# kvas7andy/unreal

Measured on NVIDIA B200. Metric: maze env-steps/s incl. pixel-change+returns, higher is better.
Workload: dtype f32

## Files before the change

include/unreal_b200.h:

```cpp
#ifndef UNREAL_B200_H_
#define UNREAL_B200_H_

#include <stdint.h>

#ifdef __cplusplus
extern "C" {
#endif

#define UNREAL_OK 0
#define UNREAL_EINVAL (-1)
#define UNREAL_ECUDA (-2)
#define UNREAL_ESTATE (-3)
#define UNREAL_ENOMEM (-4)

#define UNREAL_F32 0
#define UNREAL_U8 1
#define UNREAL_BF16 2

#define UNREAL_MAZE_GRID 7
#define UNREAL_FRAME_HW 84
#define UNREAL_PC_CELLS 20
#define UNREAL_MT_WORDS 624

const char* unreal_last_error(void);
int unreal_abi_version(void);
int unreal_device_info(int* sm_count, int* cc_major, int* cc_minor);
int unreal_set_tunable(const char* name, int value);
int unreal_get_tunable(const char* name, int* value);

int unreal_maze_set_map(const char* map49_host);
int unreal_maze_get_layout(int* start_x, int* start_y, int* goal_x, int* goal_y, uint8_t* walls49_host);

int unreal_maze_reset(int32_t* pos , int32_t* last_action , float* last_reward ,
                      const uint8_t* mask , int n, void* stream);

int unreal_maze_step(int32_t* pos, const int32_t* action , const uint8_t* active,
                     float* reward , uint8_t* terminal , int32_t* last_action,
                     float* last_reward, void* obs, int obs_dtype, float* pc, uint64_t* frame_rec,
                     int n, int auto_reset, void* stream);

int unreal_maze_window(int32_t* pos, const int32_t* action, float* reward, uint8_t* terminal, int32_t* last_action,
                       float* last_reward, void* obs, int obs_dtype, float* pc, uint64_t* frame_rec, int n, int t,
                       int auto_reset, void* stream);

int unreal_maze_render(const int32_t* pos, void* obs, int obs_dtype, int m, void* stream);

int unreal_maze_pixel_change(const int32_t* pos0, const int32_t* pos1, float* pc, int m, void* stream);
int unreal_maze_pc_targets(const int32_t* pos0, const int32_t* pos1, const int32_t* len, const float* boot, float gamma_pc,
                           float* tgt, int t, int n, void* stream);

int unreal_pixel_change(const void* cur, const void* prev, int dtype, float* pc, int m, int h, int w,
                        int c, void* stream);
int unreal_selfcheck_arith(unsigned long long* mismatches, void* stream);
int unreal_subsample(const float* a, float* out, int m, int h, int w, int width, void* stream);
int unreal_pixel_change_stream(const void* frames, int dtype, float* pc, int s, int l, int h, int w,
                               int c, void* stream);

int unreal_nstep_returns(const float* r, const float* v, const uint8_t* term, const float* boot,
                         float gamma, float* out_R, float* out_adv, int t, int n, void* stream);
int unreal_sequence_returns(const float* r, const int32_t* len, const float* boot, float gamma,
                            float* out_R , int n, int l, void* stream);

int unreal_pc_targets(const float* pc, const uint8_t* term, const int32_t* len, const float* boot,
                      float gamma_pc, float* tgt, int t, int n, void* stream);

int unreal_mt_seed(uint32_t* mt, int32_t* mt_pos, const uint32_t* seeds , int n, void* stream);
int unreal_choose_action(uint32_t* mt, int32_t* mt_pos, const float* pi, const uint8_t* active,
                         int32_t* action, int n, int a, void* stream);
int unreal_mt_randint(uint32_t* mt, int32_t* mt_pos, uint32_t high, int32_t* out, int n, int k, void* stream);

typedef struct unreal_replay unreal_replay_t;
int unreal_replay_create(unreal_replay_t** out, int n_envs, int history_size);
int unreal_replay_destroy(unreal_replay_t* r);
int unreal_replay_reset(unreal_replay_t* r, void* stream);
int unreal_replay_add(unreal_replay_t* r, const uint64_t* frame_rec , void* stream);
int unreal_replay_state(unreal_replay_t* r, uint8_t* full, int32_t* count, int64_t* top,
                        int32_t* n_pos, int32_t* n_neg, void* stream);
int unreal_replay_copy(unreal_replay_t* r, int direction, uint64_t* rec, int64_t* top, int32_t* count,
                       int32_t* n_pos, int32_t* n_neg, void* stream);
int unreal_replay_sample_sequence(unreal_replay_t* r, uint32_t* mt, int32_t* mt_pos, int seq_len,
                                  int32_t* start, int32_t* len, uint64_t* rec, void* stream);
int unreal_replay_sample_rp(unreal_replay_t* r, uint32_t* mt, int32_t* mt_pos, int32_t* start,
                            uint64_t* rec, void* stream);
int unreal_frame_unpack(const uint64_t* rec, int m, int32_t* pos0, int32_t* pos1, int32_t* action,
                        float* reward, uint8_t* terminal, int32_t* last_action, float* last_reward,
                        uint8_t* valid, void* stream);

int unreal_frame_pack(const int32_t* action, const float* reward, const uint8_t* terminal,
                      const int32_t* last_action , const float* last_reward ,
                      const uint8_t* active , uint64_t* rec, int n, void* stream);
int unreal_replay_add_slots(unreal_replay_t* r, const uint64_t* frame_rec, int32_t* slot, void* stream);
int unreal_ring_store(void* payload, const void* src, const int32_t* slot, int n_envs, int history_size,
                      long long item_bytes, void* stream);
int unreal_rows_select(void* out, const void* src, const int64_t* idx, const uint8_t* mask, int n, long long item_bytes,
                       void* stream);
int unreal_replay_gather(unreal_replay_t* r, const void* payload, long long item_bytes, const int32_t* start,
                         const int32_t* len , int seq_len, int time_major, void* out, void* stream);

int unreal_rollout_lar(const int32_t* last_action, const float* last_reward, const float* objective, int n, int a, int g,
                       float* lar, void* stream);
int unreal_rollout_post(const float* reward, const uint8_t* terminal, const uint64_t* frame_rec, int n, uint8_t* active,
                        uint8_t* ended, uint64_t* last_rec, float* episode_reward, float* lstm_c, float* lstm_h,
                        double* stats, void* stream);

int unreal_grad_sumsq(const float* grad, int64_t p, double* sumsq, void* stream);
int unreal_rmsprop_update(float* var, float* rms, float* mom, const float* grad, int64_t p,
                          const double* sumsq, float grad_scale, float lr, float decay, float momentum,
                          float eps, float clip_norm, float* grad_norm, void* stream);
int unreal_rmsprop_update_dlr(float* var, float* rms, float* mom, const float* grad, int64_t p,
                              const double* sumsq, float grad_scale, const float* lr_dev, float decay, float momentum,
                              float eps, float clip_norm, float* grad_norm, void* stream);

#define UNREAL_GEMM_OUT_F32 0
#define UNREAL_GEMM_OUT_BF16 1
int unreal_gemm_bf16(const void* a, int64_t lda, int a_mn_major, const void* b, int64_t ldb, int b_mn_major,
                     void* c, int64_t ldc, int c_dtype, const float* bias, const float* add, int relu,
                     int accumulate, int split_k, int m, int n, int k, void* stream);

int unreal_im2col(const void* in, int in_dtype, void* out_bf16, int s, int h, int w, int c, int kh, int kw,
                  int stride, void* stream);
int unreal_col2im(const void* cols, int cols_dtype, void* out, int out_dtype, const float* bias, int relu, int s,
                  int h, int w, int c, int kh, int kw, int stride, void* stream);
int unreal_lstm_cell_fwd(float* gates, const float* c_prev, float* c_out, float* h_out, void* h16_out, int n,
                         void* stream);
int unreal_lstm_cell_fwd_ld(float* gates, const float* c_prev, float* c_out, float* h_out, void* h16_out, int h16_ld,
                            int n, void* stream);
// ... 82 lines not shown
```

unreal_b200/_lib.py:

```python
import ctypes
import os
from ctypes import POINTER, c_char_p, c_double, c_float, c_int, c_int32, c_int64, c_uint8, c_uint32, c_void_p

import torch

HERE = os.path.dirname(os.path.abspath(__file__))
LIB_PATH = os.path.join(HERE, "libunreal_b200.so")

OK = 0
F32 = 0
U8 = 1


class UnrealError(RuntimeError):
  pass


if not os.path.exists(LIB_PATH):
  raise ImportError(
      "%s is missing: build it with `python -m unreal_b200.build` (nvcc, sm_100a). "
      "unreal_b200 has no CPU fallback." % LIB_PATH)

lib = ctypes.CDLL(LIB_PATH)

P = c_void_p

SIGNATURES = {
    "unreal_last_error": (c_char_p, []),
    "unreal_abi_version": (c_int, []),
    "unreal_device_info": (c_int, [POINTER(c_int), POINTER(c_int), POINTER(c_int)]),
    "unreal_set_tunable": (c_int, [c_char_p, c_int]),
    "unreal_get_tunable": (c_int, [c_char_p, POINTER(c_int)]),
    "unreal_maze_set_map": (c_int, [c_char_p]),
    "unreal_maze_get_layout": (c_int, [POINTER(c_int)] * 4 + [POINTER(c_uint8)]),
    "unreal_maze_reset": (c_int, [P, P, P, P, c_int, P]),
    "unreal_maze_step": (c_int, [P, P, P, P, P, P, P, P, c_int, P, P, c_int, c_int, P]),
    "unreal_maze_window": (c_int, [P, P, P, P, P, P, P, c_int, P, P, c_int, c_int, c_int, P]),
    "unreal_maze_render": (c_int, [P, P, c_int, c_int, P]),
    "unreal_maze_pixel_change": (c_int, [P, P, P, c_int, P]),
    "unreal_maze_pc_targets": (c_int, [P, P, P, P, c_float, P, c_int, c_int, P]),
    "unreal_pixel_change": (c_int, [P, P, c_int, P, c_int, c_int, c_int, c_int, P]),
    "unreal_pixel_change_stream": (c_int, [P, c_int, P, c_int, c_int, c_int, c_int, c_int, P]),
    "unreal_selfcheck_arith": (c_int, [P, P]),
    "unreal_subsample": (c_int, [P, P, c_int, c_int, c_int, c_int, P]),
    "unreal_nstep_returns": (c_int, [P, P, P, P, c_float, P, P, c_int, c_int, P]),
    "unreal_sequence_returns": (c_int, [P, P, P, c_float, P, c_int, c_int, P]),
    "unreal_pc_targets": (c_int, [P, P, P, P, c_float, P, c_int, c_int, P]),
    "unreal_mt_seed": (c_int, [P, P, P, c_int, P]),
    "unreal_choose_action": (c_int, [P, P, P, P, P, c_int, c_int, P]),
    "unreal_mt_randint": (c_int, [P, P, c_uint32, P, c_int, c_int, P]),
    "unreal_replay_create": (c_int, [POINTER(c_void_p), c_int, c_int]),
    "unreal_replay_destroy": (c_int, [c_void_p]),
    "unreal_replay_reset": (c_int, [c_void_p, P]),
    "unreal_replay_add": (c_int, [c_void_p, P, P]),
    "unreal_replay_state": (c_int, [c_void_p, P, P, P, P, P, P]),
    "unreal_replay_copy": (c_int, [c_void_p, c_int, P, P, P, P, P, P]),
    "unreal_replay_sample_sequence": (c_int, [c_void_p, P, P, c_int, P, P, P, P]),
    "unreal_replay_sample_rp": (c_int, [c_void_p, P, P, P, P, P]),
    "unreal_frame_unpack": (c_int, [P, c_int, P, P, P, P, P, P, P, P, P]),
    "unreal_frame_pack": (c_int, [P, P, P, P, P, P, P, c_int, P]),
    "unreal_replay_add_slots": (c_int, [c_void_p, P, P, P]),
    "unreal_ring_store": (c_int, [P, P, P, c_int, c_int, c_int64, P]),
    "unreal_rows_select": (c_int, [P, P, P, P, c_int, c_int64, P]),
    "unreal_replay_gather": (c_int, [c_void_p, P, c_int64, P, P, c_int, c_int, P, P]),
    "unreal_rollout_lar": (c_int, [P, P, P, c_int, c_int, c_int, P, P]),
    "unreal_rollout_post": (c_int, [P, P, P, c_int, P, P, P, P, P, P, P, P]),
    "unreal_grad_sumsq": (c_int, [P, c_int64, P, P]),
    "unreal_rmsprop_update": (c_int, [P, P, P, P, c_int64, P, c_float, c_float, c_float, c_float, c_float,
                                      c_float, P, P]),
    "unreal_rmsprop_update_dlr": (c_int, [P, P, P, P, c_int64, P, c_float, P, c_float, c_float, c_float,
                                          c_float, P, P]),
    "unreal_gemm_bf16": (c_int, [P, c_int64, c_int, P, c_int64, c_int, P, c_int64, c_int, P, P, c_int, c_int, c_int,
                                 c_int, c_int, c_int, P]),
    "unreal_im2col": (c_int, [P, c_int, P, c_int, c_int, c_int, c_int, c_int, c_int, c_int, P]),
    "unreal_col2im": (c_int, [P, c_int, P, c_int, P, c_int, c_int, c_int, c_int, c_int, c_int, c_int, c_int, P]),
    "unreal_lstm_cell_fwd": (c_int, [P, P, P, P, P, c_int, P]),
    "unreal_lstm_cell_fwd_ld": (c_int, [P, P, P, P, P, c_int, c_int, P]),
    "unreal_lstm_cell_act": (c_int, [P, P, P, P, P, c_int, P]),
    "unreal_lstm_cell_fwd_g16": (c_int, [P, P, P, P, P, c_int, c_int, P]),
    "unreal_lstm_cell_act_g16": (c_int, [P, P, P, P, P, c_int, P]),
    "unreal_lstm_cell_act_heads": (c_int, [P, P, P, P, c_int, P, P, P, P, c_int, P, P, P]),
    "unreal_lstm_cell_bwd_g16": (c_int, [P, P, P, P, P, P, P, c_int, P]),
    "unreal_lstm_step_fwd": (c_int, [P, c_int64, P, P, P, P, P, P, P, c_int, P, P, c_int, c_int, c_int, P]),
    "unreal_lstm_step_bwd": (c_int, [P, P, c_int64, P, P, P, P, P, P, P, c_int, c_int, P]),
    "unreal_lstm_cell_bwd": (c_int, [P, P, P, P, P, P, c_int, P]),
    "unreal_lstm_cell_bwd2": (c_int, [P, P, P, P, P, P, P, c_int, P]),
    "unreal_s2d_frames": (c_int, [P, c_int, P, c_int, P]),
    "unreal_conv_fwd": (c_int, [P, c_int, P, P, P, c_int, P]),
    "unreal_relu_grad": (c_int, [P, c_int, P, P, P, c_int64, c_int, c_int, P]),
    "unreal_conv1_wgrad": (c_int, [P, P, P, c_int, P]),
    "unreal_conv2_wgrad": (c_int, [P, P, P, c_int, P]),
    "unreal_conv2_wgrad_c8": (c_int, [P, P, P, c_int, P]),
    "unreal_conv2_dgrad": (c_int, [P, P, P, c_int, P]),
    "unreal_pc_deconv_fwd": (c_int, [P, P, P, P, c_int, P]),
    "unreal_conv2_dgrad_relu": (c_int, [P, P, P, P, P, c_int, c_int, P]),
    "unreal_conv1_wgrad_p21": (c_int, [P, P, P, c_int, P]),
    "unreal_conv1_fwd_maze": (c_int, [P, P, P, P, c_int, P]),
    "unreal_conv1_wgrad_maze": (c_int, [P, P, P, c_int, P]),
    "unreal_a3c_head_loss": (c_int, [P, P, P, P, P, P, P, P, P, c_int64, c_int, c_float, c_float, P, P, P, P, P, P]),
    "unreal_a3c_head_bwd": (c_int, [P, P, P, P, P, P, c_int64, c_int, P, P, P, P, P, P]),
    "unreal_pc_loss": (c_int, [P, P, P, P, c_int, c_float, c_int64, c_int, P, P, P, P]),
    "unreal_pc_loss_grad16": (c_int, [P, P, P, P, c_int, c_float, c_int64, c_int, P, P, P, P]),
    "unreal_cell_gather": (c_int, [P, P, P, c_int64, c_int64, c_int, P]),
    "unreal_cell_segment_sum": (c_int, [P, c_int, P, P, c_int64, c_int, P]),
    "unreal_pc_deconv_loss": (c_int, [P, P, P, P, P, P, c_int, c_float, c_int, P, P, P, P]),
    "unreal_pc_deconv_loss_c8": (c_int, [P, P, P, P, P, P, c_int, c_float, c_int, P, P, P, P]),
    "unreal_pc_deconv_loss_planes": (c_int, [P, P, P, P, P, P, c_int, c_float, c_int, P, P, P, P]),
    "unreal_pc_planes_conv": (c_int, [P, P, P, P, P, P, c_int, P]),
    "unreal_pc_planes_wgrad": (c_int, [P, P, P, c_int, P]),
    "unreal_pc_deconv_qmax": (c_int, [P, P, P, c_int, c_int, P, P]),
    "unreal_conv2_fwd_linear_scaled": (c_int, [P, P, P, P, c_int, P]),
    "unreal_conv2_fwd_linear_masked": (c_int, [P, c_int, P, P, P, P, P, c_int, P]),
    "unreal_rp_loss": (c_int, [P, P, P, c_int64, P, P, P, P, P, P]),
    "unreal_conv2_fwd_linear": (c_int, [P, P, P, c_int, P]),
}

MISSING = []
for _name, (_res, _args) in SIGNATURES.items():
  try:
    _fn = getattr(lib, _name)
# ... 83 lines not shown
```

unreal_b200/csrc/maze.cu:

```cuda
#include "common.cuh"
#include "maze_core.cuh"

namespace unreal {

__constant__ MazeLayout c_maze;
static MazeLayout h_maze;
static bool h_maze_ready = false;

static const char kReferenceMap[] =
    "--+---G"
    "--+-+++"
    "S-+---+"
    "--+++--"
    "--+-+--"
    "--+----"
    "-----++";

constexpr int kFrameElems = UNREAL_FRAME_HW * UNREAL_FRAME_HW * 3;
constexpr int kRowElems = UNREAL_FRAME_HW * 3;
constexpr int kPcElems = UNREAL_PC_CELLS * UNREAL_PC_CELLS;
constexpr int kThreads = 256;

struct StepArgs {
  int32_t* pos;
// ... 363 lines not shown
  const EnvInfo f = window_logic(a, e, t, lane);
  if (a.pc != nullptr) {
    float* pc = a.pc + b * kPcElems;
#pragma unroll
    for (int q = lane; q < kPcElems / 4; q += 32) write_pc(pc, f, q);
  }
  if (a.obs == nullptr) return;
  constexpr int G = Chunk<T>::kGroupsPerBand;
  constexpr int kChunksPerGroup = 63;
  const ChunkMasks m0 = make_masks<T>(lane);
  const ChunkMasks m1 = make_masks<T>(lane + 32);
  const bool has1 = lane + 32 < kChunksPerGroup;
  uint4* out = reinterpret_cast<uint4*>(reinterpret_cast<T*>(a.obs) + b * kFrameElems) + lane;
#pragma unroll
  for (int cy = 0; cy < UNREAL_MAZE_GRID; ++cy) {
    const uint32_t walls = c_maze.wall_rows[cy];
    const uint4 v0 = band_value(m0, walls, cy == f.ry, f.rx);
    const uint4 v1 = band_value(m1, walls, cy == f.ry, f.rx);
#pragma unroll
    for (int g = 0; g < G; ++g) {
      uint4* p = out + (size_t)(cy * G + g) * kChunksPerGroup;
      __stcs(p, v0);
      if (has1) __stcs(p + 32, v1);
    }
  }
}

template <typename T, int kWarps>
__global__ void __launch_bounds__(kWarps * 32) maze_window_env_kernel(WindowArgs a, int32_t* pos_out, int32_t* la_out,
                                                                      float* lr_out) {
  const int lane = threadIdx.x & 31;
  const int e = blockIdx.x * kWarps + (threadIdx.x >> 5);
  if (e >= a.n) return;
  constexpr int G = Chunk<T>::kGroupsPerBand;
  constexpr int kChunksPerGroup = 63;
  const ChunkMasks m0 = make_masks<T>(lane);
  const ChunkMasks m1 = make_masks<T>(lane + 32);
  const bool has1 = lane + 32 < kChunksPerGroup;
  uint4 w0[UNREAL_MAZE_GRID], w1[UNREAL_MAZE_GRID];
#pragma unroll
  for (int cy = 0; cy < UNREAL_MAZE_GRID; ++cy) {
    w0[cy] = band_value(m0, c_maze.wall_rows[cy], false, 0);
    w1[cy] = band_value(m1, c_maze.wall_rows[cy], false, 0);
  }
  const int mine = (lane < a.t) ? a.action[(size_t)lane * a.n + e] : 0;
  MazeCursor c{a.pos[2 * e], a.pos[2 * e + 1], a.last_action[e], a.last_reward[e]};
  for (int t = 0; t < a.t; ++t) {
    const int act = __shfl_sync(0xffffffffu, mine, t);
    const MazeStep st = maze_step_core(c_maze, c.x, c.y, act);
    const size_t b = (size_t)t * a.n + e;
    if (lane == 0) {
      if (a.rec) a.rec[b] = frame_pack(c.x, c.y, st.x1, st.y1, act, st.reward, st.terminal, c.la, (int)c.lr);
      a.reward[b] = (float)st.reward;
      a.terminal[b] = (uint8_t)st.terminal;
    }
    EnvInfo f;
    f.x0 = c.x; f.y0 = c.y; f.x1 = st.x1; f.y1 = st.y1; f.live = 1;
    cursor_advance(c, st, act, a.auto_reset);
    f.rx = c.x; f.ry = c.y;
    if (a.pc != nullptr) {
      float* pc = a.pc + b * kPcElems;
#pragma unroll
      for (int q = lane; q < kPcElems / 4; q += 32) write_pc(pc, f, q);
    }
    if (a.obs == nullptr) continue;
    uint4* out = reinterpret_cast<uint4*>(reinterpret_cast<T*>(a.obs) + b * kFrameElems) + lane;
    const uint4 ag0 = band_value(m0, 0u, true, f.rx), ag1 = band_value(m1, 0u, true, f.rx);
#pragma unroll
    for (int cy = 0; cy < UNREAL_MAZE_GRID; ++cy) {
      uint4 v0 = w0[cy], v1 = w1[cy];
      if (cy == f.ry) {
        v0.x |= ag0.x; v0.y |= ag0.y; v0.z |= ag0.z; v0.w |= ag0.w;
        v1.x |= ag1.x; v1.y |= ag1.y; v1.z |= ag1.z; v1.w |= ag1.w;
      }
#pragma unroll
      for (int g = 0; g < G; ++g) {
        uint4* p = out + (size_t)(cy * G + g) * kChunksPerGroup;
        __stcs(p, v0);
        if (has1) __stcs(p + 32, v1);
      }
    }
  }
  if (lane == 0) { pos_out[2 * e] = c.x; pos_out[2 * e + 1] = c.y; la_out[e] = c.la; lr_out[e] = c.lr; }
}

template <bool kStep>
__global__ void __launch_bounds__(256) maze_s2d_kernel(StepArgs a) {
  __shared__ EnvInfo s_info;
  const int tid = threadIdx.x;
  const int e = blockIdx.x;
  if (tid == 0) s_info = env_logic<kStep>(a, e);
  __syncthreads();
  const EnvInfo f = s_info;
  if (!f.live) return;
  if (a.pc != nullptr && tid >= 256 - kPcElems / 4) write_pc(a.pc + (size_t)e * kPcElems, f, tid - (256 - kPcElems / 4));
  if (a.obs == nullptr) return;
  uint4* out = reinterpret_cast<uint4*>(a.obs) + (size_t)e * (6 * 441);
  int kind[2];
#pragma unroll
  for (int h = 0; h < 2; ++h) {
    const int pix = tid + h * 256;
    const int Y = pix / 21, X = pix - Y * 21;
    const int cx = X / 3, cy = Y / 3;
    kind[h] = pix < 441 ? (int)((c_maze.wall_rows[cy] >> cx) & 1u) | (((cx == f.rx) && (cy == f.ry)) ? 2 : 0) : -1;
  }
#pragma unroll
  for (int q = 0; q < 6; ++q) {
    const int base = (2 * q) % 3;
    uint32_t wl[4], ag[4];
#pragma unroll
    for (int k = 0; k < 4; ++k) {
      const int c0 = (base + 2 * k) % 3, c1 = (base + 2 * k + 1) % 3;
      wl[k] = (c0 == 0 ? 0x3f80u : 0u) | (c1 == 0 ? 0x3f800000u : 0u);
      ag[k] = (c0 == 1 ? 0x3f80u : 0u) | (c1 == 1 ? 0x3f800000u : 0u);
    }
#pragma unroll
    for (int h = 0; h < 2; ++h) {
      if (kind[h] < 0) continue;
      const uint32_t mw = (kind[h] & 1) ? 0xffffffffu : 0u, ma = (kind[h] & 2) ? 0xffffffffu : 0u;
      __stcs(out + q * 441 + tid + h * 256, make_uint4((wl[0] & mw) | (ag[0] & ma), (wl[1] & mw) | (ag[1] & ma),
                                                       (wl[2] & mw) | (ag[2] & ma), (wl[3] & mw) | (ag[3] & ma)));
    }
  }
}

__global__ void __launch_bounds__(128) maze_pc_pairs_kernel(const int32_t* __restrict__ p0,
                                                            const int32_t* __restrict__ p1, float* pc, int m) {
  int idx = blockIdx.x * blockDim.x + threadIdx.x;
  int e = idx / (kPcElems / 4), q = idx - e * (kPcElems / 4);
  if (e >= m) return;
  EnvInfo f;
  f.x0 = p0[2 * e]; f.y0 = p0[2 * e + 1]; f.x1 = p1[2 * e]; f.y1 = p1[2 * e + 1];
  f.rx = f.ry = 0; f.live = 1;
  write_pc(pc + (size_t)e * kPcElems, f, q);
}

__global__ void __launch_bounds__(128) maze_pc_targets_kernel(const int2* __restrict__ p0, const int2* __restrict__ p1,
                                                              const int32_t* __restrict__ len, const float4* __restrict__ boot,
                                                              float g, float4* __restrict__ tgt, int T, int N) {
  const size_t per_t = (size_t)N * (kPcElems / 4);
  const size_t idx = (size_t)blockIdx.x * 128 + threadIdx.x;
  if (idx >= per_t) return;
  const int n = (int)(idx / (kPcElems / 4)), q = (int)(idx - (size_t)n * (kPcElems / 4));
  const int n_t = len ? max(0, min(len[n], T)) : T;
  const float4 zero = make_float4(0.f, 0.f, 0.f, 0.f);
  float4 R = boot[idx];
  for (int t = T - 1; t >= n_t; --t) __stcs(tgt + (size_t)t * per_t + idx, zero);
#pragma unroll 4
  for (int t = n_t - 1; t >= 0; --t) {
    const int2 a = __ldg(p0 + (size_t)t * N + n), b = __ldg(p1 + (size_t)t * N + n);
    const float4 pc = pc_value4(a.x, a.y, b.x, b.y, q);
    R.x = __fadd_rn(pc.x, __fmul_rn(g, R.x));
    R.y = __fadd_rn(pc.y, __fmul_rn(g, R.y));
    R.z = __fadd_rn(pc.z, __fmul_rn(g, R.z));
    R.w = __fadd_rn(pc.w, __fmul_rn(g, R.w));
    __stcs(tgt + (size_t)t * per_t + idx, R);
  }
}

__global__ void maze_reset_kernel(int32_t* pos, int32_t* last_action, float* last_reward, const uint8_t* mask,
                                  int n) {
  int e = blockIdx.x * blockDim.x + threadIdx.x;
  if (e >= n || (mask != nullptr && mask[e] == 0)) return;
  pos[2 * e] = c_maze.start_x;
  pos[2 * e + 1] = c_maze.start_y;
  if (last_action) last_action[e] = 0;
// ... 140 lines not shown
  if (rc) return rc;
  StepArgs a{pos, action, active, reward, terminal, last_action, last_reward, obs, pc, frame_rec, n, auto_reset};
  return launch_render<true>(a, obs_dtype, as_stream(stream));
}

extern "C" int unreal_maze_render(const int32_t* pos, void* obs, int obs_dtype, int m, void* stream) {
  UNREAL_REQUIRE(pos && obs && m >= 0, "unreal_maze_render: null argument or m < 0");
  UNREAL_REQUIRE(obs_dtype == UNREAL_F32 || obs_dtype == UNREAL_U8 || obs_dtype == UNREAL_BF16,
                 "unreal_maze_render: bad obs_dtype %d", obs_dtype);
  UNREAL_REQUIRE(aligned16(obs), "unreal_maze_render: obs must be 16-byte aligned");
  int rc = ensure_map();
  if (rc) return rc;
  StepArgs a{const_cast<int32_t*>(pos), nullptr, nullptr, nullptr, nullptr, nullptr, nullptr, obs, nullptr, nullptr, m, 0};
  return launch_render<false>(a, obs_dtype, as_stream(stream));
}

extern "C" int unreal_maze_pixel_change(const int32_t* pos0, const int32_t* pos1, float* pc, int m, void* stream) {
  UNREAL_REQUIRE(pos0 && pos1 && pc && m >= 0, "unreal_maze_pixel_change: null argument or m < 0");
  UNREAL_REQUIRE(aligned16(pc), "unreal_maze_pixel_change: pc must be 16-byte aligned");
  if (m == 0) return UNREAL_OK;
  long long threads = (long long)m * (kPcElems / 4);
  maze_pc_pairs_kernel<<<(unsigned)((threads + 127) / 128), 128, 0, as_stream(stream)>>>(pos0, pos1, pc, m);
  UNREAL_LAUNCH_CHECK("maze_pc_pairs_kernel");
  return UNREAL_OK;
}

extern "C" int unreal_maze_pc_targets(const int32_t* pos0, const int32_t* pos1, const int32_t* len, const float* boot,
                                      float gamma_pc, float* tgt, int t, int n, void* stream) {
  UNREAL_REQUIRE(t >= 0 && n >= 0, "unreal_maze_pc_targets: negative size");
  if (t == 0 || n == 0) return UNREAL_OK;
  UNREAL_REQUIRE(pos0 && pos1 && boot && tgt, "unreal_maze_pc_targets: pos0, pos1, boot and tgt must be non-null");
  UNREAL_REQUIRE(aligned16(boot) && aligned16(tgt) && (reinterpret_cast<uintptr_t>(pos0) & 7u) == 0 &&
                 (reinterpret_cast<uintptr_t>(pos1) & 7u) == 0, "unreal_maze_pc_targets: alignment (16 bytes; cells 8)");
  const long long cols = (long long)n * (kPcElems / 4);
  maze_pc_targets_kernel<<<(unsigned)((cols + 127) / 128), 128, 0, as_stream(stream)>>>(
      reinterpret_cast<const int2*>(pos0), reinterpret_cast<const int2*>(pos1), len, reinterpret_cast<const float4*>(boot),
      gamma_pc, reinterpret_cast<float4*>(tgt), t, n);
  UNREAL_LAUNCH_CHECK("maze_pc_targets_kernel");
  return UNREAL_OK;
}

extern "C" int unreal_maze_window(int32_t* pos, const int32_t* action, float* reward, uint8_t* terminal, int32_t* last_action,
                                  float* last_reward, void* obs, int obs_dtype, float* pc, uint64_t* frame_rec, int n, int t,
                                  int auto_reset, void* stream) {
  UNREAL_REQUIRE(n >= 0 && t >= 0, "unreal_maze_window: negative size");
  UNREAL_REQUIRE(t <= 32, "unreal_maze_window: at most 32 steps per window (got %d)", t);
  UNREAL_REQUIRE(pos && action && reward && terminal && last_action && last_reward,
                 "unreal_maze_window: pos/action/reward/terminal/last_action/last_reward must be non-null");
  UNREAL_REQUIRE(obs_dtype == UNREAL_F32 || obs_dtype == UNREAL_U8, "unreal_maze_window: obs_dtype must be f32 or u8");
  UNREAL_REQUIRE(aligned16(obs) && aligned16(pc), "unreal_maze_window: obs and pc must be 16-byte aligned");
  UNREAL_REQUIRE((long long)n * t < 2147483647LL / 4, "unreal_maze_window: window too large for one launch");
  int rc = ensure_map();
  if (rc) return rc;
  if (n == 0 || t == 0) return UNREAL_OK;
  cudaStream_t st = as_stream(stream);
  WindowArgs a{pos, last_action, last_reward, action, reward, terminal, obs, pc, frame_rec, n, t, auto_reset};
  const long long items = (long long)n * t;
  int variant = get_tunable("maze_render_variant", -1);
  if (variant < 0 || variant == 1) variant = (obs == nullptr || obs_dtype == UNREAL_U8) ? 3 : 0;
  if (variant == 3) {
    const int warps = get_tunable("maze_warps_per_cta", 8);
    if (obs_dtype == UNREAL_F32) maze_window_env_kernel<float, 4><<<(n + 3) / 4, 128, 0, st>>>(a, pos, last_action, last_reward);
    else if (warps == 4) maze_window_env_kernel<uint8_t, 4><<<(n + 3) / 4, 128, 0, st>>>(a, pos, last_action, last_reward);
    else if (warps == 2) maze_window_env_kernel<uint8_t, 2><<<(n + 1) / 2, 64, 0, st>>>(a, pos, last_action, last_reward);
    else if (warps == 1) maze_window_env_kernel<uint8_t, 1><<<n, 32, 0, st>>>(a, pos, last_action, last_reward);
    else maze_window_env_kernel<uint8_t, 8><<<(n + 7) / 8, 256, 0, st>>>(a, pos, last_action, last_reward);
    UNREAL_LAUNCH_CHECK("maze_window_env_kernel");
    return UNREAL_OK;
  }
  if (variant == 2) {
    if (obs_dtype == UNREAL_F32) maze_window_warp_kernel<float, 4><<<(unsigned)((items + 3) / 4), 128, 0, st>>>(a);
    else if (get_tunable("maze_warps_per_cta", 4) == 8) maze_window_warp_kernel<uint8_t, 8><<<(unsigned)((items + 7) / 8), 256, 0, st>>>(a);
    else maze_window_warp_kernel<uint8_t, 4><<<(unsigned)((items + 3) / 4), 128, 0, st>>>(a);
    UNREAL_LAUNCH_CHECK("maze_window_warp_kernel");
  } else {
    if (obs_dtype == UNREAL_F32) maze_window_cta_kernel<float, 256><<<(unsigned)items, 256, 0, st>>>(a);
    else maze_window_cta_kernel<uint8_t, 256><<<(unsigned)items, 256, 0, st>>>(a);
    UNREAL_LAUNCH_CHECK("maze_window_cta_kernel");
  }
  maze_window_state_kernel<<<(n + 127) / 128, 128, 0, st>>>(pos, last_action, last_reward, action, n, t, auto_reset);
  UNREAL_LAUNCH_CHECK("maze_window_state_kernel");
  return UNREAL_OK;
}
```

unreal_b200/kernels.py:

```python
import ctypes

import torch

from . import _lib
from ._lib import call, ptr, stream_ptr

FRAME = 84
PC = 20
MT_WORDS = 624


def maze_set_map(map49=None):
  call("unreal_maze_set_map", None if map49 is None else map49.encode())


def maze_layout():
  v = [ctypes.c_int() for _ in range(4)]
  walls = (ctypes.c_uint8 * 49)()
  call("unreal_maze_get_layout", *[ctypes.byref(x) for x in v], walls)
  return (v[0].value, v[1].value), (v[2].value, v[3].value), bytes(walls)


class MazeState(object):

  def __init__(self, n, device):
    self.n = n
    self.device = torch.device(device)
    self.pos = torch.zeros(n, 2, dtype=torch.int32, device=device)
    self.last_action = torch.zeros(n, dtype=torch.int32, device=device)
    self.last_reward = torch.zeros(n, dtype=torch.float32, device=device)
    maze_reset(self)


def maze_reset(state, mask=None):
  call("unreal_maze_reset", ptr(state.pos, torch.int32), ptr(state.last_action, torch.int32),
       ptr(state.last_reward, torch.float32), ptr(mask, torch.uint8), state.n, stream_ptr())


def maze_step(state, action, obs=None, pc=None, reward=None, terminal=None, frame_rec=None, active=None,
              auto_reset=False):
  n = state.n
  dev = state.device
  if reward is None:
    reward = torch.empty(n, dtype=torch.float32, device=dev)
  if terminal is None:
    terminal = torch.empty(n, dtype=torch.uint8, device=dev)
  cell_obs = obs if (obs is not None and obs.dtype == torch.int32) else None
  if cell_obs is not None:
    if cell_obs.numel() != n * 2:
      raise _lib.UnrealError("an int32 (cell) observation buffer must hold [N,2]")
    obs = None
  if obs is not None and obs.numel() != n * FRAME * FRAME * 3:
    raise _lib.UnrealError("obs must hold [N,84,84,3]")
  if pc is not None and (pc.numel() != n * PC * PC or pc.dtype != torch.float32):
    raise _lib.UnrealError("pc must be float32 [N,20,20]")
  call("unreal_maze_step", ptr(state.pos, torch.int32), ptr(action, torch.int32, "action"),
       ptr(active, torch.uint8, "active"), ptr(reward, torch.float32), ptr(terminal, torch.uint8),
       ptr(state.last_action, torch.int32), ptr(state.last_reward, torch.float32),
       ptr(obs), _lib.dtype_tag(obs) if obs is not None else _lib.F32, ptr(pc),
       ptr(frame_rec, torch.int64, "frame_rec"), n, 1 if auto_reset else 0, stream_ptr())
  if cell_obs is not None:
    if active is None:
      cell_obs.copy_(state.pos.view_as(cell_obs))
    else:
      co = cell_obs.view(n, 2)
      torch.where(active.view(n, 1).bool(), state.pos.view(n, 2), co, out=co)
  return reward, terminal


def maze_window(state, actions, obs=None, pc=None, reward=None, terminal=None, frame_rec=None, auto_reset=False):
  t, n = actions.shape
  dev = state.device
  if n != state.n:
    raise _lib.UnrealError("actions must be [T, %d]" % state.n)
  if reward is None:
    reward = torch.empty(t, n, dtype=torch.float32, device=dev)
  if terminal is None:
    terminal = torch.empty(t, n, dtype=torch.uint8, device=dev)
  if obs is not None and (obs.numel() != t * n * FRAME * FRAME * 3 or obs.dtype not in (torch.float32, torch.uint8)):
    raise _lib.UnrealError("obs must hold [T,N,84,84,3] float32 or uint8")
  if pc is not None and (pc.numel() != t * n * PC * PC or pc.dtype != torch.float32):
    raise _lib.UnrealError("pc must be float32 [T,N,20,20]")
  call("unreal_maze_window", ptr(state.pos, torch.int32), ptr(actions, torch.int32, "actions"), ptr(reward, torch.float32),
       ptr(terminal, torch.uint8), ptr(state.last_action, torch.int32), ptr(state.last_reward, torch.float32), ptr(obs),
       _lib.dtype_tag(obs) if obs is not None else _lib.F32, ptr(pc), ptr(frame_rec, torch.int64, "frame_rec"), n, t,
       1 if auto_reset else 0, stream_ptr())
  return reward, terminal


def obs_shape(dtype):
  if dtype == torch.int32:
    return (2,)
  return (6, 441, 8) if dtype == torch.bfloat16 else (FRAME, FRAME, 3)


def maze_render(pos, out=None, dtype=torch.float32):
  m = pos.shape[0]
  if (out is not None and out.dtype == torch.int32) or (out is None and dtype == torch.int32):
    if out is None:
      return pos.reshape(m, 2).clone()
    out.copy_(pos.view_as(out))
    return out
  if out is None:
    out = torch.empty(m, *obs_shape(dtype), dtype=dtype, device=pos.device)
  call("unreal_maze_render", ptr(pos, torch.int32, "pos"), ptr(out), _lib.dtype_tag(out), m, stream_ptr())
  return out


def maze_pixel_change(pos0, pos1, out=None):
  m = pos0.shape[0]
  if out is None:
    out = torch.empty(m, PC, PC, dtype=torch.float32, device=pos0.device)
  call("unreal_maze_pixel_change", ptr(pos0, torch.int32), ptr(pos1, torch.int32), ptr(out, torch.float32), m,
       stream_ptr())
  return out


def maze_pc_targets(pos0, pos1, length, boot, gamma_pc, out=None):
  t, n = pos0.shape[0], pos0.shape[1]
  if out is None:
    out = torch.empty(t, n, PC, PC, dtype=torch.float32, device=pos0.device)
  call("unreal_maze_pc_targets", ptr(pos0, torch.int32), ptr(pos1, torch.int32), ptr(length, torch.int32),
       ptr(boot, torch.float32), float(gamma_pc), ptr(out, torch.float32), t, n, stream_ptr())
  return out


def pixel_change(cur, prev, out=None):
  m, h, w, c = cur.shape
  if out is None:
    out = torch.empty(m, (h - 4) // 4, (w - 4) // 4, dtype=torch.float32, device=cur.device)
  if prev.shape != cur.shape or prev.dtype != cur.dtype:
    raise _lib.UnrealError("cur and prev must have the same shape and dtype")
  call("unreal_pixel_change", ptr(cur), ptr(prev), _lib.dtype_tag(cur), ptr(out, torch.float32), m, h, w, c,
       stream_ptr())
  return out


def pixel_change_stream(frames, out=None):
  s, l1, h, w, c = frames.shape
  if out is None:
    out = torch.empty(s, l1 - 1, (h - 4) // 4, (w - 4) // 4, dtype=torch.float32, device=frames.device)
  call("unreal_pixel_change_stream", ptr(frames), _lib.dtype_tag(frames), ptr(out, torch.float32), s, l1 - 1, h, w,
       c, stream_ptr())
  return out


def selfcheck_arith():
  out = torch.zeros(2, dtype=torch.int64, device="cuda")
  call("unreal_selfcheck_arith", ptr(out), stream_ptr())
  return tuple(int(x) for x in out.tolist())


def subsample(a, width, out=None):
  m, h, w = a.shape
  if out is None:
    out = torch.empty(m, h // width, w // width, dtype=torch.float32, device=a.device)
  call("unreal_subsample", ptr(a, torch.float32, "a"), ptr(out, torch.float32, "out"), m, h, w, int(width), stream_ptr())
  return out


def nstep_returns(r, v, term, boot, gamma, out_R=None, out_adv=None):
  t, n = r.shape
  if out_R is None:
    out_R = torch.empty_like(r)
  if v is not None and out_adv is None:
    out_adv = torch.empty_like(r)
  call("unreal_nstep_returns", ptr(r, torch.float32), ptr(v, torch.float32), ptr(term, torch.uint8),
       ptr(boot, torch.float32), float(gamma), ptr(out_R, torch.float32), ptr(out_adv, torch.float32), t, n,
       stream_ptr())
  return out_R, out_adv


# ... 714 lines not shown
```

unreal_b200/train/rollout.py:

```python
import torch

from .. import _lib
from .. import kernels as K


class RolloutTargets(object):
  def __init__(self, num_envs, rollout_len=20, gamma=0.99, gamma_pc=0.9, obs_dtype=torch.float32,
               device="cuda:0", auto_reset=True, use_graphs=True, window_kernel=None):
    self.n = int(num_envs)
    self.t = int(rollout_len)
    self.gamma = float(gamma)
    self.gamma_pc = float(gamma_pc)
    self.device = torch.device(device)
    self.auto_reset = auto_reset
    self.use_graphs = use_graphs
    self.window_kernel = (self.t <= 32) if window_kernel is None else bool(window_kernel)
    if self.window_kernel and self.t > 32:
      raise _lib.UnrealError("the window kernel covers at most 32 rollout steps")
    d, n, t = self.device, self.n, self.t
    with torch.cuda.device(d):
      self.state = K.MazeState(n, d)
    self.actions = torch.zeros(t, n, dtype=torch.int32, device=d)
    self.values = torch.zeros(t, n, dtype=torch.float32, device=d)
    self.boot_value = torch.zeros(n, dtype=torch.float32, device=d)
    self.boot_q = torch.zeros(n, 20, 20, dtype=torch.float32, device=d)
    self.obs = torch.empty(t, n, 84, 84, 3, dtype=obs_dtype, device=d)
    self.pc = torch.empty(t, n, 20, 20, dtype=torch.float32, device=d)
    self.reward = torch.empty(t, n, dtype=torch.float32, device=d)
    self.terminal = torch.empty(t, n, dtype=torch.uint8, device=d)
    self.frame_rec = torch.empty(t, n, dtype=torch.int64, device=d)
    self.R = torch.empty(t, n, dtype=torch.float32, device=d)
    self.adv = torch.empty(t, n, dtype=torch.float32, device=d)
    self.pc_tgt = torch.empty(t, n, 20, 20, dtype=torch.float32, device=d)
    self._graphs = None
    self._h_in = None
    self._h_out = None
    self._copy_stream = None
    self.host_graph = True
    self._host_graph = None

  @property
  def launches_per_pass(self):
    return ((1 if self.obs.dtype == torch.uint8 else 2) if self.window_kernel else self.t) + 2

  def _steps(self):
    if self.window_kernel:
      K.maze_window(self.state, self.actions, obs=self.obs, pc=self.pc, reward=self.reward, terminal=self.terminal,
                    frame_rec=self.frame_rec, auto_reset=self.auto_reset)
      return
    for t in range(self.t):
      K.maze_step(self.state, self.actions[t], obs=self.obs[t], pc=self.pc[t], reward=self.reward[t],
                  terminal=self.terminal[t], frame_rec=self.frame_rec[t], auto_reset=self.auto_reset)

  def _returns(self):
    K.nstep_returns(self.reward, self.values, self.terminal, self.boot_value, self.gamma, self.R, self.adv)

  def _pc_targets(self):
    K.pc_targets(self.pc, self.terminal, None, self.boot_q, self.gamma_pc, self.pc_tgt)

  def _capture(self):
    torch.cuda.synchronize(self.device)
    self._steps(); self._returns(); self._pc_targets()
    K.maze_reset(self.state)
    torch.cuda.synchronize(self.device)
    graphs = []
    for fn in (self._steps, self._returns, self._pc_targets):
      g = torch.cuda.CUDAGraph()
      with _lib.graph_capture(g):
        fn()
      graphs.append(g)
    self._graphs = graphs

  def run_device(self, events=None):
    with torch.cuda.device(self.device):
      if self.use_graphs and self._graphs is None:
        self._capture()
      phases = ([g.replay for g in self._graphs] if self.use_graphs
                else [self._steps, self._returns, self._pc_targets])
      if events is not None:
        events[0].record()
      for i, ph in enumerate(phases):
        ph()
        if events is not None:
          events[i + 1].record()

  def _ensure_host(self):
    if self._h_in is None:
      t, n = self.t, self.n
      pin = dict(pin_memory=True)
      self._h_in = dict(actions=torch.zeros(t, n, dtype=torch.int32, **pin),
                        values=torch.zeros(t, n, dtype=torch.float32, **pin),
                        boot_value=torch.zeros(n, dtype=torch.float32, **pin),
                        boot_q=torch.zeros(n, 20, 20, dtype=torch.float32, **pin))
      self._h_out = dict(reward=torch.zeros(t, n, dtype=torch.float32, **pin),
                         terminal=torch.zeros(t, n, dtype=torch.uint8, **pin),
                         R=torch.zeros(t, n, dtype=torch.float32, **pin),
                         adv=torch.zeros(t, n, dtype=torch.float32, **pin))

  @property
  def h2d_bytes_per_pass(self):
    self._ensure_host()
    return sum(v.numel() * v.element_size() for v in self._h_in.values())

  @property
  def d2h_bytes_per_pass(self):
    self._ensure_host()
    return sum(v.numel() * v.element_size() for v in self._h_out.values())

  def host_inputs(self):
    self._ensure_host()
    return {k: v.numpy() for k, v in self._h_in.items()}

  def run_host(self, actions=None, values=None, boot_value=None, boot_q=None):
    self._ensure_host()
    hi, ho = self._h_in, self._h_out
    for name, arr in (("actions", actions), ("values", values), ("boot_value", boot_value), ("boot_q", boot_q)):
      if arr is None:
        continue
      t = torch.as_tensor(arr)
      if t.data_ptr() != hi[name].data_ptr():
        hi[name].copy_(t)
    with torch.cuda.device(self.device):
      if self.use_graphs and self._graphs is None:
        self._capture()
      if self._copy_stream is None:
        self._copy_stream = torch.cuda.Stream(self.device)
        self._ev = [torch.cuda.Event() for _ in range(5)]
      main = torch.cuda.current_stream()
      if self.use_graphs and self.host_graph:
        if self._host_graph is None:
          self._pipeline(main)
          main.synchronize()
          g = torch.cuda.CUDAGraph()
          with _lib.graph_capture(g):
            self._pipeline(torch.cuda.current_stream(), replay_graphs=False)
          self._host_graph = g
        else:
          self._host_graph.replay()
      else:
        self._pipeline(main)
      main.synchronize()
    return {k: v.numpy() for k, v in self._h_out.items()}

  def _pipeline(self, main, replay_graphs=True):
    hi, ho = self._h_in, self._h_out
    side = self._copy_stream
    ev_start, ev_in, ev_k1, ev_k3, ev_out = self._ev
    phases = ([g.replay for g in self._graphs] if (self.use_graphs and replay_graphs)
              else [self._steps, self._returns, self._pc_targets])
    ev_start.record(main)
    self.actions.copy_(hi["actions"], non_blocking=True)
    side.wait_event(ev_start)
    with torch.cuda.stream(side):
      self.values.copy_(hi["values"], non_blocking=True)
      self.boot_value.copy_(hi["boot_value"], non_blocking=True)
      self.boot_q.copy_(hi["boot_q"], non_blocking=True)
      ev_in.record(side)
    phases[0]()
    ev_k1.record(main)
    with torch.cuda.stream(side):
      side.wait_event(ev_k1)
      ho["reward"].copy_(self.reward, non_blocking=True)
      ho["terminal"].copy_(self.terminal, non_blocking=True)
    main.wait_event(ev_in)
    phases[1]()
    ev_k3.record(main)
    with torch.cuda.stream(side):
# ... 7 lines not shown
```

Measured before the change: 78.43 million.

## Capture all rollout phases in one CUDA graph and add fused maze pass kernel

```diff
diff --git a/include/unreal_b200.h b/include/unreal_b200.h
--- a/include/unreal_b200.h
+++ b/include/unreal_b200.h
@@ -42,6 +42,11 @@
 int unreal_maze_window(int32_t* pos, const int32_t* action, float* reward, uint8_t* terminal, int32_t* last_action,
                        float* last_reward, void* obs, int obs_dtype, float* pc, uint64_t* frame_rec, int n, int t,
                        int auto_reset, void* stream);
+
+int unreal_maze_pass(int32_t* pos, int32_t* last_action, float* last_reward, const int32_t* action, const float* values,
+                     const float* boot_value, const float* boot_q, float gamma, float gamma_pc, int auto_reset, void* obs,
+                     int obs_dtype, float* pc, float* reward, uint8_t* terminal, uint64_t* frame_rec, float* R,
+                     float* adv, float* pc_tgt, int32_t* arrivals, int n, int t, void* stream);
 
 int unreal_maze_render(const int32_t* pos, void* obs, int obs_dtype, int m, void* stream);
 
diff --git a/unreal_b200/_lib.py b/unreal_b200/_lib.py
--- a/unreal_b200/_lib.py
+++ b/unreal_b200/_lib.py
@@ -36,6 +36,8 @@
     "unreal_maze_reset": (c_int, [P, P, P, P, c_int, P]),
     "unreal_maze_step": (c_int, [P, P, P, P, P, P, P, P, c_int, P, P, c_int, c_int, P]),
     "unreal_maze_window": (c_int, [P, P, P, P, P, P, P, c_int, P, P, c_int, c_int, c_int, P]),
+    "unreal_maze_pass": (c_int, [P, P, P, P, P, P, P, c_float, c_float, c_int, P, c_int, P, P, P, P, P, P, P, P, c_int,
+                                 c_int, P]),
     "unreal_maze_render": (c_int, [P, P, c_int, c_int, P]),
     "unreal_maze_pixel_change": (c_int, [P, P, P, c_int, P]),
     "unreal_maze_pc_targets": (c_int, [P, P, P, P, c_float, P, c_int, c_int, P]),
diff --git a/unreal_b200/csrc/maze.cu b/unreal_b200/csrc/maze.cu
--- a/unreal_b200/csrc/maze.cu
+++ b/unreal_b200/csrc/maze.cu
@@ -469,6 +469,165 @@
     }
   }
   if (lane == 0) { pos_out[2 * e] = c.x; pos_out[2 * e + 1] = c.y; la_out[e] = c.la; lr_out[e] = c.lr; }
+}
+
+struct PassArgs {
+  int32_t* pos;
+  int32_t* last_action;
+  float* last_reward;
+  const int32_t* action;
+  const float* values;
+  const float* boot_value;
+  const float4* boot_q;
+  void* obs;
+  float4* pc;
+  float* reward;
+  uint8_t* terminal;
+  uint64_t* rec;
+  float* R;
+  float* adv;
+  float4* pc_tgt;
+  int32_t* arrivals;
+  float gamma, gamma_pc;
+  int n, t, steps, auto_reset;
+};
+
+template <typename T, int kVec> struct PassShape;
+template <> struct PassShape<float, 16> { static constexpr int kGroups = 12, kRows = 4; };
+template <> struct PassShape<float, 32> { static constexpr int kGroups = 6, kRows = 3; };
+template <> struct PassShape<uint8_t, 16> { static constexpr int kGroups = 3, kRows = 3; };
+
+template <typename T, int kVec>
+constexpr int pass_threads() { return (PassShape<T, kVec>::kRows * 63 + 31) / 32 * 32; }
+
+template <int kVec> struct Chunkv { uint4 h[kVec / 16]; };
+__device__ __forceinline__ void store_cs(uint8_t* p, const Chunkv<16>& v) { __stcs(reinterpret_cast<uint4*>(p), v.h[0]); }
+__device__ __forceinline__ void store_cs(uint8_t* p, const Chunkv<32>& v) {
+  asm volatile("st.global.cs.v8.b32 [%0], {%1, %2, %3, %4, %5, %6, %7, %8};" ::"l"(p), "r"(v.h[0].x), "r"(v.h[0].y),
+               "r"(v.h[0].z), "r"(v.h[0].w), "r"(v.h[1].x), "r"(v.h[1].y), "r"(v.h[1].z), "r"(v.h[1].w)
+               : "memory");
+}
+
+__device__ __forceinline__ int pass_cell(int p, int k) { return (p >> (3 * k)) & 7; }
+__device__ __forceinline__ int pass_terminal(int p) { return (p >> 18) & 1; }
+__device__ __forceinline__ int pass_reward(int p) { return ((p >> 19) & 3) - 1; }
+
+template <typename T, int kVec>
+__global__ void __launch_bounds__(pass_threads<T, kVec>()) maze_pass_kernel(PassArgs a) {
+  using Shape = PassShape<T, kVec>;
+  constexpr int kThreads = pass_threads<T, kVec>();
+  constexpr int kUsed = Shape::kRows * 63;
+  constexpr int kHalves = kVec / 16;
+  constexpr uint32_t kFull = 0xffffffffu;
+  const int tid = threadIdx.x, lane = tid & 31, warp = tid >> 5;
+  const int n = a.n;
+  const int blk = blockIdx.x / n, e = blockIdx.x - blk * n;
+  const int t0 = blk * a.steps, t1 = min(a.t, t0 + a.steps);
+
+  const int act_l = lane < a.t ? __ldg(a.action + (size_t)lane * n + e) : 0;
+  MazeCursor c{a.pos[2 * e], a.pos[2 * e + 1], a.last_action[e], a.last_reward[e]};
+  int info = 0, la_l = 0, lr_l = 0;
+  for (int s = 0; s < a.t; ++s) {
+    const int act = __shfl_sync(kFull, act_l, s);
+    const MazeStep st = maze_step_core(c_maze, c.x, c.y, act);
+    const int p = c.x | (c.y << 3) | (st.x1 << 6) | (st.y1 << 9) | (st.terminal << 18) | ((st.reward + 1) << 19);
+    if (lane == s) { info = p; la_l = c.la; lr_l = (int)c.lr; }
+    cursor_advance(c, st, act, a.auto_reset);
+    if (lane == s) info |= (c.x << 12) | (c.y << 15);
+  }
+  if (lane == 0) {
+    __threadfence();
+    const int arrivals = (int)(gridDim.x / n) * (kThreads / 32);
+    if (atomicAdd(a.arrivals + e, 1) == arrivals - 1) {
+      a.pos[2 * e] = c.x; a.pos[2 * e + 1] = c.y; a.last_action[e] = c.la; a.last_reward[e] = c.lr;
+      a.arrivals[e] = 0;
+    }
+  }
+
+  if (warp == kThreads / 32 - 1) {
+    const float rew = (float)pass_reward(info);
+    float R = a.boot_value[e], mine = 0.f;
+    for (int s = a.t - 1; s >= t0; --s) {
+      const float r = __shfl_sync(kFull, rew, s);
+      R = __shfl_sync(kFull, pass_terminal(info), s) ? 0.f : R;
+      R = __fadd_rn(r, __fmul_rn(a.gamma, R));
+      if (lane == s) mine = R;
+    }
+    if (lane >= t0 && lane < t1) {
+      const size_t b = (size_t)lane * n + e;
+      a.reward[b] = rew;
+      a.terminal[b] = (uint8_t)pass_terminal(info);
+      a.R[b] = mine;
+      a.adv[b] = __fsub_rn(mine, a.values[b]);
+      if (a.rec) a.rec[b] = frame_pack(pass_cell(info, 0), pass_cell(info, 1), pass_cell(info, 2), pass_cell(info, 3),
+                                       act_l, pass_reward(info), pass_terminal(info), la_l, lr_l);
+    }
+  }
+
+  if (warp < (kPcElems / 4 + 31) / 32) {
+    const int q = tid;
+    const float4 zero = make_float4(0.f, 0.f, 0.f, 0.f);
+    float4 R = q < kPcElems / 4 ? a.boot_q[(size_t)e * (kPcElems / 4) + q] : zero;
+    for (int s = a.t - 1; s >= t0; --s) {
+      const int p = __shfl_sync(kFull, info, s);
+      if (q < kPcElems / 4) {
+        const float4 v = pc_value4(pass_cell(p, 0), pass_cell(p, 1), pass_cell(p, 2), pass_cell(p, 3), q);
+        if (pass_terminal(p)) R = zero;
+        R.x = __fadd_rn(v.x, __fmul_rn(a.gamma_pc, R.x));
+        R.y = __fadd_rn(v.y, __fmul_rn(a.gamma_pc, R.y));
+        R.z = __fadd_rn(v.z, __fmul_rn(a.gamma_pc, R.z));
+        R.w = __fadd_rn(v.w, __fmul_rn(a.gamma_pc, R.w));
+        if (s < t1) {
+          const size_t o = ((size_t)s * n + e) * (kPcElems / 4) + q;
+          __stcs(a.pc_tgt + o, R);
+          if (a.pc) __stcs(a.pc + o, v);
+        }
+      }
+    }
+  }
+
+  if (a.obs == nullptr) return;
+  const int gsub = tid / 63, col = tid - gsub * 63;
+  Chunkv<kVec> wall[UNREAL_MAZE_GRID];
+  uint4 agA[kHalves], agB[kHalves];
+  int cxA[kHalves], cxB[kHalves];
+#pragma unroll
+  for (int h = 0; h < kHalves; ++h) {
+    const ChunkMasks m = make_masks<T>(col * kHalves + h);
+#pragma unroll
+    for (int cy = 0; cy < UNREAL_MAZE_GRID; ++cy) wall[cy].h[h] = band_value(m, c_maze.wall_rows[cy], false, 0);
+    agA[h] = band_value(m, 0u, true, m.cxA);
+    agB[h] = band_value(m, 0u, true, m.cxB);
+    cxA[h] = m.cxA; cxB[h] = m.cxB;
+  }
+  constexpr size_t kFrameBytes = (size_t)kFrameElems * sizeof(T);
+  constexpr size_t kBandStride = (size_t)63 * kVec;
+  for (int s = t0; s < t1; ++s) {
+    const int p = __shfl_sync(kFull, info, s);
+    if (tid >= kUsed) continue;
+    const int rx = pass_cell(p, 4), ry = pass_cell(p, 5);
+    Chunkv<kVec> ag;
+#pragma unroll
+    for (int h = 0; h < kHalves; ++h) {
+      const uint32_t ma = cxA[h] == rx ? kFull : 0u, mb = cxB[h] == rx ? kFull : 0u;
+      ag.h[h] = make_uint4((agA[h].x & ma) | (agB[h].x & mb), (agA[h].y & ma) | (agB[h].y & mb),
+                           (agA[h].z & ma) | (agB[h].z & mb), (agA[h].w & ma) | (agB[h].w & mb));
+    }
+    uint8_t* out = reinterpret_cast<uint8_t*>(a.obs) + ((size_t)s * n + e) * kFrameBytes + (size_t)tid * kVec;
+#pragma unroll
+    for (int cy = 0; cy < UNREAL_MAZE_GRID; ++cy) {
+      Chunkv<kVec> v = wall[cy];
+      if (cy == ry) {
+#pragma unroll
+        for (int h = 0; h < kHalves; ++h) {
+          v.h[h].x |= ag.h[h].x; v.h[h].y |= ag.h[h].y; v.h[h].z |= ag.h[h].z; v.h[h].w |= ag.h[h].w;
+        }
+      }
+#pragma unroll
+      for (int i = 0; i < Shape::kGroups / Shape::kRows; ++i)
+        store_cs(out + (size_t)(cy * Shape::kGroups + Shape::kRows * i) * kBandStride, v);
+    }
+  }
 }
 
 template <bool kStep>
@@ -775,3 +934,41 @@
   UNREAL_LAUNCH_CHECK("maze_window_state_kernel");
   return UNREAL_OK;
 }
+
+extern "C" int unreal_maze_pass(int32_t* pos, int32_t* last_action, float* last_reward, const int32_t* action,
+                                const float* values, const float* boot_value, const float* boot_q, float gamma,
+                                float gamma_pc, int auto_reset, void* obs, int obs_dtype, float* pc, float* reward,
+                                uint8_t* terminal, uint64_t* frame_rec, float* R, float* adv, float* pc_tgt,
+                                int32_t* arrivals, int n, int t, void* stream) {
+  UNREAL_REQUIRE(n >= 0 && t >= 0, "unreal_maze_pass: negative size");
+  UNREAL_REQUIRE(t <= 32, "unreal_maze_pass: at most 32 steps per pass (got %d)", t);
+  UNREAL_REQUIRE(pos && last_action && last_reward && action && values && boot_value && boot_q && reward && terminal &&
+                 R && adv && pc_tgt && arrivals,
+                 "unreal_maze_pass: only obs, pc and frame_rec may be null");
+  UNREAL_REQUIRE(obs_dtype == UNREAL_F32 || obs_dtype == UNREAL_U8, "unreal_maze_pass: obs_dtype must be f32 or u8");
+  UNREAL_REQUIRE(aligned16(obs) && aligned16(pc) && aligned16(boot_q) && aligned16(pc_tgt) &&
+                 (reinterpret_cast<uintptr_t>(frame_rec) & 7u) == 0,
+                 "unreal_maze_pass: obs, pc, boot_q and pc_tgt must be 16-byte aligned, frame_rec 8-byte aligned");
+  UNREAL_REQUIRE((long long)n * t < 2147483647LL / 4, "unreal_maze_pass: pass too large for one launch");
+  int rc = ensure_map();
+  if (rc) return rc;
+  if (n == 0 || t == 0) return UNREAL_OK;
+  int steps = get_tunable("maze_pass_steps", 0);
+  if (steps <= 0) steps = obs_dtype == UNREAL_F32 ? 2 : 5;
+  steps = min(steps, t);
+  const int blocks = (t + steps - 1) / steps;
+  PassArgs a{pos, last_action, last_reward, action, values, boot_value, reinterpret_cast<const float4*>(boot_q), obs,
+             reinterpret_cast<float4*>(pc), reward, terminal, frame_rec, R, adv, reinterpret_cast<float4*>(pc_tgt),
+             arrivals, gamma, gamma_pc, n, t, steps, auto_reset};
+  const unsigned grid = (unsigned)blocks * (unsigned)n;
+  cudaStream_t st = as_stream(stream);
+  if (obs_dtype == UNREAL_U8) {
+    maze_pass_kernel<uint8_t, 16><<<grid, pass_threads<uint8_t, 16>(), 0, st>>>(a);
+  } else if (get_tunable("maze_pass_store_bytes", 16) == 32 && (reinterpret_cast<uintptr_t>(obs) & 31u) == 0) {
+    maze_pass_kernel<float, 32><<<grid, pass_threads<float, 32>(), 0, st>>>(a);
+  } else {
+    maze_pass_kernel<float, 16><<<grid, pass_threads<float, 16>(), 0, st>>>(a);
+  }
+  UNREAL_LAUNCH_CHECK("maze_pass_kernel");
+  return UNREAL_OK;
+}
diff --git a/unreal_b200/kernels.py b/unreal_b200/kernels.py
--- a/unreal_b200/kernels.py
+++ b/unreal_b200/kernels.py
@@ -88,6 +88,29 @@
   return reward, terminal
 
 
+def maze_pass(state, actions, values, boot_value, boot_q, gamma, gamma_pc, arrivals, reward, terminal, R, adv, pc_tgt,
+              obs=None, pc=None, frame_rec=None, auto_reset=False):
+  t, n = actions.shape
+  if n != state.n:
+    raise _lib.UnrealError("actions must be [T, %d]" % state.n)
+  if obs is not None and (obs.numel() != t * n * FRAME * FRAME * 3 or obs.dtype not in (torch.float32, torch.uint8)):
+    raise _lib.UnrealError("obs must hold [T,N,84,84,3] float32 or uint8")
+  for name, x, count in (("values", values, t * n), ("boot_value", boot_value, n), ("boot_q", boot_q, n * PC * PC),
+                         ("reward", reward, t * n), ("R", R, t * n), ("adv", adv, t * n),
+                         ("pc_tgt", pc_tgt, t * n * PC * PC), ("pc", pc, t * n * PC * PC)):
+    if x is not None and x.numel() != count:
+      raise _lib.UnrealError("%s must hold %d elements" % (name, count))
+  if terminal.numel() != t * n or arrivals.numel() != n or (frame_rec is not None and frame_rec.numel() != t * n):
+    raise _lib.UnrealError("terminal / frame_rec must hold [T,N], arrivals [N]")
+  call("unreal_maze_pass", ptr(state.pos, torch.int32), ptr(state.last_action, torch.int32),
+       ptr(state.last_reward, torch.float32), ptr(actions, torch.int32, "actions"), ptr(values, torch.float32, "values"),
+       ptr(boot_value, torch.float32, "boot_value"), ptr(boot_q, torch.float32, "boot_q"), float(gamma),
+       float(gamma_pc), 1 if auto_reset else 0, ptr(obs), _lib.dtype_tag(obs) if obs is not None else _lib.F32,
+       ptr(pc, torch.float32, "pc"), ptr(reward, torch.float32, "reward"), ptr(terminal, torch.uint8, "terminal"),
+       ptr(frame_rec, torch.int64, "frame_rec"), ptr(R, torch.float32, "R"), ptr(adv, torch.float32, "adv"),
+       ptr(pc_tgt, torch.float32, "pc_tgt"), ptr(arrivals, torch.int32, "arrivals"), n, t, stream_ptr())
+
+
 def obs_shape(dtype):
   if dtype == torch.int32:
     return (2,)
diff --git a/unreal_b200/train/rollout.py b/unreal_b200/train/rollout.py
--- a/unreal_b200/train/rollout.py
+++ b/unreal_b200/train/rollout.py
@@ -33,6 +33,7 @@
     self.adv = torch.empty(t, n, dtype=torch.float32, device=d)
     self.pc_tgt = torch.empty(t, n, 20, 20, dtype=torch.float32, device=d)
     self._graphs = None
+    self._pass_graph = None
     self._h_in = None
     self._h_out = None
     self._copy_stream = None
@@ -70,12 +71,16 @@
         fn()
       graphs.append(g)
     self._graphs = graphs
+    self._pass_graph = torch.cuda.CUDAGraph()
+    with _lib.graph_capture(self._pass_graph):
+      for fn in (self._steps, self._returns, self._pc_targets):
+        fn()
 
   def run_device(self, events=None):
     with torch.cuda.device(self.device):
       if self.use_graphs and self._graphs is None:
         self._capture()
-      phases = ([g.replay for g in self._graphs] if self.use_graphs
+      phases = ([self._pass_graph.replay] if self.use_graphs
                 else [self._steps, self._returns, self._pc_targets])
       if events is not None:
         events[0].record()
@@ -83,6 +88,9 @@
         ph()
         if events is not None:
           events[i + 1].record()
+      if events is not None:
+        for ev in events[len(phases) + 1:]:
+          ev.record()
 
   def _ensure_host(self):
     if self._h_in is None:
```

Measured after the change: 78.73 million (median of 6 runs). About the same (+0.4%).
